# SAR-Research-Lab/lvt

Hardware: AMD Instinct MI355X
Metric: stereo frames/sec (KITTI-shaped 1241x376), per-frame SE3 vs CPU ref (higher is better)
Workload: dtype u8/f64

## Files before the change

include/lvt_amd_ext.h:

```cpp
#ifndef LVT_AMD_EXT_H__
#define LVT_AMD_EXT_H__

#include "lvt_c.h"
#include <stdint.h>

#ifdef __cplusplus
extern "C" {
#endif

typedef struct lvt_amd_params {
    float fx, fy, cx, cy;
    float baseline;
    int img_width, img_height;
    float k1, k2, p1, p2, k3;
    float near_plane_distance, far_plane_distance;
    float triangulation_ratio_test_threshold;
    float tracking_ratio_test_threshold;
    float descriptor_matching_threshold;
    int min_num_matches_for_tracking;
    int tracking_radius;
    int detection_cell_size;
    int max_keypoints_per_cell;
    int agast_threshold;
    int untracked_threshold;
// ... 34 lines not shown
LVT_API void lvt_amd_batch_track_device_async(lvt_handle h, const void *const *d_left, const void *const *d_right,
                                              int n_rows, int n_cols, int pitch_bytes);
LVT_API void lvt_amd_batch_wait(lvt_handle h, double *R, double *t, int *status);
LVT_API void lvt_amd_batch_get_counts(lvt_handle h, int seq, int out[32]);
LVT_API lvt_handle lvt_amd_batch_create_mixed(const lvt_amd_params *p , int sensor_type, int n_sequences);
LVT_API int lvt_amd_batch_track_device_async_mixed(lvt_handle h, const void *const *d_left, const void *const *d_right,
                                                   const int *n_rows, const int *n_cols, const int *pitch_bytes);
LVT_API int lvt_amd_batch_get_params(lvt_handle h, int seq, lvt_amd_params *out);
LVT_API int lvt_amd_batch_mixed_tables(const lvt_amd_params *p, int sensor_type, int n_sequences, unsigned *cells, int cells_cap,
                                       unsigned *score, int score_cap, int counts[2]);

LVT_API void lvt_amd_set_stream(lvt_handle h, void *hip_stream);
LVT_API const char *lvt_amd_last_error(lvt_handle h);

LVT_API void lvt_amd_get_host_stats(lvt_handle h, long long out[8]);

LVT_API void lvt_amd_profile_enable(lvt_handle h, int enable);
LVT_API int lvt_amd_profile_read(lvt_handle h, int slot, char *name, int name_cap, double *total_ms, long *calls);

enum {
    LVT_AMD_C_N_LEFT = 0, LVT_AMD_C_N_RIGHT, LVT_AMD_C_MAP_SIZE, LVT_AMD_C_STAGED_SIZE, LVT_AMD_C_N_MATCHES,
    LVT_AMD_C_SECOND_PASS, LVT_AMD_C_N_ROW_MATCHES, LVT_AMD_C_N_TRIANGULATED, LVT_AMD_C_TRIANGULATED,
    LVT_AMD_C_RETRY_LEFT, LVT_AMD_C_RETRY_RIGHT, LVT_AMD_C_PNP_ITERS, LVT_AMD_C_PNP_INLIERS,
    LVT_AMD_C_MAP_SIZE_AT_MATCH, LVT_AMD_C_N_STAGED_ERASED, LVT_AMD_C_N_STAGED_PROMOTED, LVT_AMD_C_N_CULLED,
    LVT_AMD_C_FRAME, LVT_AMD_C_OVERFLOW ,
    LVT_AMD_C_PNP_BORDERLINE ,
    LVT_AMD_C_ROW_FALLBACK ,
    LVT_AMD_C_PNP_TRIALS , LVT_AMD_C_PNP_REJECTIONS ,
    LVT_AMD_C_PNP_TERMINATES ,
    LVT_AMD_C__COUNT = 32
};
LVT_API void lvt_amd_get_counts(lvt_handle h, int out[LVT_AMD_C__COUNT]);
LVT_API int lvt_amd_get_features(lvt_handle h, int eye, float *xy, float *resp, uint8_t *desc, int cap);
LVT_API int lvt_amd_get_matches(lvt_handle h, int *feat_idx, double *xyz, int cap);
LVT_API int lvt_amd_get_row_matches(lvt_handle h, int *pairs, int cap);
LVT_API int lvt_amd_get_map(lvt_handle h, double *xyz, int *counter, int *age, uint8_t *desc, int cap);
LVT_API int lvt_amd_get_staged(lvt_handle h, double *xyz, int *counter, uint8_t *desc, int cap);
enum { LVT_AMD_LISTS_MAP = 0, LVT_AMD_LISTS_STAGED = 1, LVT_AMD_LISTS_ROW = 2 };
typedef struct {
    int kc;
    int stood_down_map;
    int stood_down_row;
    int pass2;
    int n_early;
    int binned;
    int n;
    int reserved;
} lvt_amd_list_info;
LVT_API int lvt_amd_get_candidate_lists(lvt_handle h, int which, unsigned *keys, int *counts, float *proj, signed char *vis, int cap, lvt_amd_list_info *info);
LVT_API void lvt_amd_get_pose(lvt_handle h, double q_wxyz[4], double p[3]);
LVT_API int lvt_amd_get_last_pose(lvt_handle h, double q_wxyz[4], double p[3]);
LVT_API void lvt_amd_get_predicted_pose(lvt_handle h, double q_wxyz[4], double p[3]);
LVT_API void lvt_amd_get_debug(lvt_handle h, long long out[32]);
LVT_API void lvt_amd_get_timeline(lvt_handle h, long long out[16]);
LVT_API int lvt_amd_get_ordering(lvt_handle h);
LVT_API int lvt_amd_get_plane(lvt_handle h, int eye, int what, void *dst, int cap_bytes, int *pitch_out);

LVT_API int lvt_amd_pnp(const lvt_amd_params *p, const double q_in[4], const double p_in[3], const double *pts,
                        const float *obs, int n, double q_out[4], double p_out[3], int *n_solve_calls);
LVT_API int lvt_amd_pnp_detail(const lvt_amd_params *p, const double q_in[4], const double p_in[3], const double *pts,
                               const float *obs, int n, double q_out[4], double p_out[3], int *n_solve_calls,
                               double *err_out, int *level_out, int *borderline);
LVT_API int lvt_amd_pnp_trace(const lvt_amd_params *p, const double q_in[4], const double p_in[3], const double *pts,
                              const float *obs, int n, double q_out[4], double p_out[3], int *n_solve_calls,
                              double *err_out, int *level_out, int *borderline, double *trace, int trace_cap, int stats[3]);
LVT_API int lvt_amd_motion_predict(double state[14], const double q[4], const double p[3], double q_out[4], double p_out[3]);
// ... 177 lines not shown
```

lvt_amd/__init__.py:

```python
from __future__ import annotations

import ctypes as C
import os

import numpy as np

from .params import LvtParameters, ParamsPOD, kitti_params, euroc_params, tum_params

_HERE = os.path.dirname(os.path.abspath(__file__))
LIB_PATH = os.environ.get("LVT_AMD_LIB") or os.path.join(_HERE, "lib", "liblvt_c.so")

ABI_SYMBOLS = [
    "lvt_create", "lvt_destroy", "lvt_track", "lvt_track_with_external_corners", "lvt_get_status",
    "lvt_amd_default_params", "lvt_amd_params_from_file", "lvt_amd_create", "lvt_amd_reset",
    "lvt_amd_track_rgbd", "lvt_amd_track_device", "lvt_amd_track_device_async", "lvt_amd_wait",
    "lvt_amd_set_stream", "lvt_amd_last_error", "lvt_amd_get_counts", "lvt_amd_get_features",
    "lvt_amd_get_matches", "lvt_amd_get_row_matches", "lvt_amd_get_map", "lvt_amd_get_staged", "lvt_amd_get_candidate_lists",
    "lvt_amd_get_pose", "lvt_amd_get_last_pose", "lvt_amd_get_predicted_pose", "lvt_amd_get_plane", "lvt_amd_pnp", "lvt_amd_pnp_detail",
    "lvt_amd_hamming_match_batched", "lvt_amd_hamming_match_batched_n", "lvt_amd_rectifier_create", "lvt_amd_rectifier_destroy",
    "lvt_amd_rectify_device", "lvt_amd_rectify", "lvt_amd_rectifier_get_maps",
    "lvt_amd_odometry_create", "lvt_amd_odometry_destroy", "lvt_amd_odometry_reset", "lvt_amd_odometry_push_pose", "lvt_amd_odometry_update", "lvt_amd_profile_enable", "lvt_amd_profile_read", "lvt_amd_get_debug", "lvt_amd_get_timeline", "lvt_amd_get_ordering",
    "lvt_amd_batch_create", "lvt_amd_batch_size", "lvt_amd_batch_track_device_async", "lvt_amd_batch_wait",
    "lvt_amd_batch_get_counts", "lvt_amd_create_on_device", "lvt_amd_get_device", "lvt_amd_wait_status", "lvt_amd_get_host_stats",
    "lvt_amd_track_async", "lvt_amd_track_rgbd_async", "lvt_amd_pnp_trace", "lvt_amd_create_pooled", "lvt_amd_wait_pose",
    "lvt_amd_batch_create_mixed", "lvt_amd_batch_track_device_async_mixed", "lvt_amd_batch_get_params", "lvt_amd_batch_mixed_tables",
    "lvt_amd_track_rgbd_device", "lvt_amd_track_rgbd_device_async", "lvt_amd_track_rgbd16", "lvt_amd_track_rgbd16_async",
    "lvt_amd_batch_track_rgbd_device_async",
    "lvt_amd_set_rectifiers", "lvt_amd_batch_set_rectifiers",
    "lvt_amd_set_pixel_format", "lvt_amd_batch_set_pixel_format", "lvt_amd_get_pixel_format",
    "lvt_amd_motion_predict",
    "lvt_amd_snapshot_take", "lvt_amd_snapshot_apply", "lvt_amd_batch_snapshot_take", "lvt_amd_batch_snapshot_apply", "lvt_amd_snapshot_get_info",
    "lvt_amd_snapshot_get_params", "lvt_amd_snapshot_export", "lvt_amd_snapshot_import", "lvt_amd_snapshot_describe", "lvt_amd_snapshot_destroy",
    "lvt_amd_batch_reset",
    "lvt_amd_enable_pose_info", "lvt_amd_get_pose_info", "lvt_amd_pose_info_eval", "lvt_amd_pose_info_to_ros",
    "lvt_amd_odometry_push_pose_cov", "lvt_amd_odometry_update_cov",
    "lvt_amd_set_depth_camera", "lvt_amd_batch_set_depth_camera", "lvt_amd_get_depth_camera", "lvt_amd_register_depth_device",
    "lvt_amd_set_equalisation", "lvt_amd_batch_set_equalisation", "lvt_amd_get_equalisation", "lvt_amd_equalise_device", "lvt_amd_equalisation_plan",
    "lvt_amd_set_mask", "lvt_amd_batch_set_mask", "lvt_amd_set_mask_device", "lvt_amd_batch_set_mask_device", "lvt_amd_get_mask_stats", "lvt_amd_mask_features",
    "lvt_amd_set_label_mask", "lvt_amd_batch_set_label_mask", "lvt_amd_get_label_mask", "lvt_amd_frame_labels", "lvt_amd_frame_labels_device", "lvt_amd_build_label_mask",
    "lvt_amd_depth_guard_default", "lvt_amd_set_depth_guard", "lvt_amd_batch_set_depth_guard", "lvt_amd_get_depth_guard", "lvt_amd_get_depth_guard_stats", "lvt_amd_depth_guard_features",
    "lvt_amd_relocalise", "lvt_amd_batch_relocalise", "lvt_amd_odometry_set_relocalisation", "lvt_amd_reloc_default_config", "lvt_amd_reloc_slice_length", "lvt_amd_reloc_match_device", "lvt_amd_reloc_solve", "lvt_amd_reloc_correspond",
]

N_COUNTS = 32
COUNT_NAMES = ["n_left", "n_right", "map_size", "staged_size", "n_matches", "second_pass", "n_row_matches",
               "n_triangulated", "triangulated", "retry_left", "retry_right", "pnp_iters", "pnp_inliers",
               "map_size_at_match", "n_staged_erased", "n_staged_promoted", "n_culled", "frame", "overflow", "pnp_borderline", "row_fallback", "pnp_trials", "pnp_rejections", "pnp_terminates"]

LISTS_WHICH = {"map": 0, "staged": 1, "row": 2}
LIST_INFO_NAMES = ["kc", "stood_down_map", "stood_down_row", "pass2", "n_early", "binned", "n"]

eState_NOT_INITIALIZED, eState_TRACKING, eState_LOST = 1, 2, 3
eSensor_STEREO, eSensor_RGBD = 1, 2
PIX_GRAY8, PIX_BGR8, PIX_RGB8, PIX_BGRA8, PIX_RGBA8 = 0, 1, 2, 3, 4
PIX_BPP = {PIX_GRAY8: 1, PIX_BGR8: 3, PIX_RGB8: 3, PIX_BGRA8: 4, PIX_RGBA8: 4}
DEPTH_F32, DEPTH_U16 = 0, 1

_lib = None


def load_library():
    global _lib
    if _lib is not None:
        return _lib
    if not os.path.exists(LIB_PATH):
        raise RuntimeError(f"{LIB_PATH} is missing: build it with `make -C lvt_amd/csrc` "
                           "(there is no CPU fallback for the tracking path)")
    try:
        import torch
    except Exception:
        pass
    L = C.CDLL(LIB_PATH)
    vp = C.c_void_p
    L.lvt_create.restype = vp
    L.lvt_create.argtypes = [C.c_char_p, C.c_int]
    L.lvt_amd_create.restype = vp
    L.lvt_amd_create.argtypes = [vp, C.c_int]
    L.lvt_amd_create_on_device.restype = vp
    L.lvt_amd_create_on_device.argtypes = [vp, C.c_int, C.c_int]
    L.lvt_amd_get_device.argtypes = [vp]
    L.lvt_amd_create_pooled.restype = vp
    L.lvt_amd_create_pooled.argtypes = [vp, C.c_int, C.c_int]
    L.lvt_destroy.argtypes = [vp]
    L.lvt_amd_reset.argtypes = [vp]
    L.lvt_track.argtypes = [vp, vp, vp, C.c_int, C.c_int, vp, vp]
    L.lvt_track_with_external_corners.argtypes = [vp, vp, vp, C.c_int, C.c_int, vp, C.c_int, vp, C.c_int, vp, vp]
    L.lvt_get_status.argtypes = [vp]
    L.lvt_amd_params_from_file.argtypes = [C.c_char_p, vp]
    L.lvt_amd_default_params.argtypes = [vp]
    L.lvt_amd_track_rgbd.argtypes = [vp, vp, vp, C.c_int, C.c_int, vp, vp]
    L.lvt_amd_track_device.argtypes = [vp, vp, vp, C.c_int, C.c_int, C.c_int, vp, vp]
    L.lvt_amd_track_device_async.argtypes = [vp, vp, vp, C.c_int, C.c_int, C.c_int]
    L.lvt_amd_wait.argtypes = [vp, vp, vp]
    L.lvt_amd_track_async.argtypes = [vp, vp, vp, C.c_int, C.c_int]
    L.lvt_amd_track_async.restype = C.c_int
    L.lvt_amd_track_rgbd_async.argtypes = [vp, vp, vp, C.c_int, C.c_int]
    L.lvt_amd_track_rgbd_async.restype = C.c_int
    L.lvt_amd_wait_status.argtypes = [vp, vp, vp]
    L.lvt_amd_wait_status.restype = C.c_int
    L.lvt_amd_set_stream.argtypes = [vp, vp]
    L.lvt_amd_last_error.restype = C.c_char_p
    L.lvt_amd_last_error.argtypes = [vp]
    L.lvt_amd_get_counts.argtypes = [vp, vp]
    L.lvt_amd_get_features.argtypes = [vp, C.c_int, vp, vp, vp, C.c_int]
    L.lvt_amd_get_matches.argtypes = [vp, vp, vp, C.c_int]
    L.lvt_amd_get_row_matches.argtypes = [vp, vp, C.c_int]
    L.lvt_amd_get_map.argtypes = [vp, vp, vp, vp, vp, C.c_int]
    L.lvt_amd_get_staged.argtypes = [vp, vp, vp, vp, C.c_int]
    L.lvt_amd_get_candidate_lists.argtypes = [vp, C.c_int, vp, vp, vp, vp, C.c_int, vp]
    L.lvt_amd_get_candidate_lists.restype = C.c_int
    L.lvt_amd_get_pose.argtypes = [vp, vp, vp]
    L.lvt_amd_get_last_pose.argtypes = [vp, vp, vp]
    L.lvt_amd_get_predicted_pose.argtypes = [vp, vp, vp]
    L.lvt_amd_get_plane.argtypes = [vp, C.c_int, C.c_int, vp, C.c_int, vp]
    L.lvt_amd_pnp.argtypes = [vp, vp, vp, vp, vp, C.c_int, vp, vp, vp]
    L.lvt_amd_pnp_detail.argtypes = [vp, vp, vp, vp, vp, C.c_int, vp, vp, vp, vp, vp, vp]
    L.lvt_amd_pnp_trace.argtypes = [vp, vp, vp, vp, vp, C.c_int, vp, vp, vp, vp, vp, vp, vp, C.c_int, vp]
    L.lvt_amd_motion_predict.argtypes = [vp, vp, vp, vp, vp]
    L.lvt_amd_motion_predict.restype = C.c_int
    L.lvt_amd_hamming_match_batched.restype = C.c_float
    L.lvt_amd_hamming_match_batched.argtypes = [vp, vp, vp, vp, vp, C.c_int, C.c_int, C.c_int, C.c_float, C.c_int, C.c_int, C.c_int, vp, vp]
    L.lvt_amd_get_timeline.argtypes = [vp, vp]
    L.lvt_amd_get_ordering.argtypes = [vp]
    L.lvt_amd_get_ordering.restype = C.c_int
    L.lvt_amd_rectifier_create.restype = vp
    L.lvt_amd_rectifier_create.argtypes = [vp, vp, vp, vp, C.c_int, C.c_int]
    L.lvt_amd_rectifier_destroy.argtypes = [vp]
    L.lvt_amd_rectify_device.argtypes = [vp, vp, C.c_int, vp, C.c_int, vp]
    L.lvt_amd_rectify.argtypes = [vp, vp, vp]
    L.lvt_amd_rectifier_get_maps.argtypes = [vp, vp, vp]
    L.lvt_amd_odometry_create.restype = vp
    L.lvt_amd_odometry_create.argtypes = [vp, vp, C.c_int]
    L.lvt_amd_odometry_destroy.argtypes = [vp]
    L.lvt_amd_odometry_reset.argtypes = [vp]
    L.lvt_amd_odometry_push_pose.restype = C.c_int
    L.lvt_amd_odometry_push_pose.argtypes = [vp, vp, vp, C.c_int, C.c_double, vp, vp]
    L.lvt_amd_odometry_update.restype = C.c_int
# ... 813 lines not shown
        return _depth_guard_of(self._h, 0)

    def depth_guard_stats(self):
        return _depth_guard_stats_of(self._h, 0)

    def _depth(self, d):
        want = getattr(self, "_depth_shape", None)
        if want is not None and tuple(d.shape) != want:
            raise ValueError(f"a depth image of shape {tuple(d.shape)} on a system whose depth camera delivers {want}")
        return d

    def depth_camera(self):
        return _depth_camera_of(self._h, 0)

    def enable_pose_info(self, on: bool = True) -> int:
        return load_library().lvt_amd_enable_pose_info(self._h, 1 if on else 0)

    def pose_info(self) -> PoseInfo:
        return _pose_info_of(self._h, 0)

    def set_stream(self, hip_stream: int):
        load_library().lvt_amd_set_stream(self._h, C.c_void_p(hip_stream))

    def counts(self):
        a = np.zeros(N_COUNTS, dtype=np.int32)
        load_library().lvt_amd_get_counts(self._h, _p(a))
        return {n: int(a[i]) for i, n in enumerate(COUNT_NAMES)}

    def features(self, eye=0, cap=16384):
        xy = np.zeros((cap, 2), np.float32); resp = np.zeros(cap, np.float32); desc = np.zeros((cap, 32), np.uint8)
        n = load_library().lvt_amd_get_features(self._h, eye, _p(xy), _p(resp), _p(desc), cap)
        return xy[:n].copy(), resp[:n].copy(), desc[:n].copy()

    def matches(self, cap=65536):
        fi = np.zeros(cap, np.int32); xyz = np.zeros((cap, 3), np.float64)
        n = load_library().lvt_amd_get_matches(self._h, _p(fi), _p(xyz), cap)
        return fi[:n].copy(), xyz[:n].copy()

    def row_matches(self, cap=16384):
        pr = np.zeros((cap, 2), np.int32)
        n = load_library().lvt_amd_get_row_matches(self._h, _p(pr), cap)
        return pr[:n].copy()

    def map(self, cap=65536):
        xyz = np.zeros((cap, 3)); cnt = np.zeros(cap, np.int32); age = np.zeros(cap, np.int32); desc = np.zeros((cap, 32), np.uint8)
        n = load_library().lvt_amd_get_map(self._h, _p(xyz), _p(cnt), _p(age), _p(desc), cap)
        return xyz[:n].copy(), cnt[:n].copy(), age[:n].copy(), desc[:n].copy()

    def staged(self, cap=65536):
        xyz = np.zeros((cap, 3)); cnt = np.zeros(cap, np.int32); desc = np.zeros((cap, 32), np.uint8)
        n = load_library().lvt_amd_get_staged(self._h, _p(xyz), _p(cnt), _p(desc), cap)
        return xyz[:n].copy(), cnt[:n].copy(), desc[:n].copy()

    def candidate_lists(self, which, cap=None):
        w = LISTS_WHICH[which] if isinstance(which, str) else int(which)
        L = load_library()
        info = np.zeros(8, np.int32)
        if cap is None:
            L.lvt_amd_get_candidate_lists(self._h, w, None, None, None, None, 0, _p(info))
            cap = int(info[6])
        kc = 128
        keys = np.zeros((max(cap, 1), kc), np.uint32); counts = np.zeros(max(cap, 1), np.int32)
        proj = np.zeros((max(cap, 1), 2), np.float32); vis = np.zeros(max(cap, 1), np.int8)
        n = L.lvt_amd_get_candidate_lists(self._h, w, _p(keys), _p(counts), _p(proj), _p(vis), cap, _p(info))
        if n < 0:
            raise ValueError("lvt_amd_get_candidate_lists refused the call (bad handle, a batch, `which` out of range, or cap too small)")
# ... 407 lines not shown
```

lvt_amd/csrc/k_features.hip:

```cpp
#include "lvt_dev.h"
#include "lvt_handover.h"
#include "lvt_math.h"
#include <type_traits>

namespace lvt {

__constant__ signed char c_brief[256][4] = {
#include "../../include/lvt_brief256_pattern.inc"
};
constexpr signed char BRIEF_TABLE[256][4] = {
#include "../../include/lvt_brief256_pattern.inc"
};
constexpr int brief_max_offset() {
    int m = 0;
    for (int i = 0; i < 256; i++)
        for (int k = 0; k < 4; k++) m = (BRIEF_TABLE[i][k] > m) ? BRIEF_TABLE[i][k] : (-BRIEF_TABLE[i][k] > m) ? -BRIEF_TABLE[i][k] : m;
    return m;
}

constexpr int TS_W = 64, TS_H = 16, HALO = 4;
constexpr int TILE_W = TS_W + 2 * HALO;
constexpr int TILE_H = TS_H + 2 * HALO;

typedef short s16x2 __attribute__((ext_vector_type(2)));
// ... 1621 lines not shown
    const int n_out = anms_select<uint16_t>(S, c.g, L, n, out, nullptr);
    cell_finish(FB, eye, cell, 0, n_out);
}

__device__ __forceinline__ bool brief_border_keep(float x, float y, int rows, int cols) {
    const int B = 28;
    if (rows <= 2 * B || cols <= 2 * B) return false;
    const int ix = __float2int_rn(x), iy = __float2int_rn(y);
    return ix >= B && ix < cols - B && iy >= B && iy < rows - B;
}

template <bool BV>
__global__ __launch_bounds__(1024) void k_gather(SeqArg<BV> sa, int par) {
    const Seq &S = sa.get();
    const int eye = blockIdx.y;
    const FrameBuf &FB = S.fb[par];
    FeatCtl &ctl = *FB.fc;
    extern __shared__ __attribute__((aligned(16))) uint8_t smem[];
    const CellLds L = carve_cell_lds(smem);
    int *cell_off = L.row_first;
    int *scan = L.scan;
    const int tid = threadIdx.x;
    const Feat &F = FB.feat[eye];
    if (ctl.poison) return;
    if (!ctl.ext_corners && !(eye == 1 && S.prm.sensor == 2) && ctl.n_detected[eye] < CORNERS_LOW_TH) {
        for (int cell = 0; cell < S.prm.n_cells; cell++) {
            cells_work(S, FB, eye, cell, 1, L);
            __syncthreads();
        }
        __builtin_amdgcn_fence(__ATOMIC_RELEASE, "workgroup");
        __syncthreads();
        __builtin_amdgcn_fence(__ATOMIC_ACQUIRE, "workgroup");
    }
    if (eye == 1 && S.prm.sensor == 2) {
        if (tid == 0) *F.n = 0;
        return;
    }
    const FrameIn &in = ctl.in;
    const bool rgbd = (S.prm.sensor == 2);
    const float *ext_xy = nullptr, *depth_img = nullptr;
    int depth_pitch = 0, depth_format = DEPTH_F32;
    float depth_scale = 0.f;
    if (ctl.ext_corners) ext_xy = wave_uniform(in.ext_xy[eye]);
    if (rgbd) {
        depth_img = wave_uniform(in.depth_img);
        depth_pitch = wave_uniform(in.depth_pitch), depth_format = wave_uniform(in.depth_format);
        depth_scale = wave_uniform(in.depth_scale);
    }
    const int nc = ctl.ext_corners ? 1 : S.prm.n_cells;
    if (tid == 0) {
        int acc = 0;
        for (int c = 0; c < nc; c++) {
            cell_off[c] = acc;
            acc += ctl.ext_corners ? ctl.n_ext[eye] : FB.cell_n[eye][c];
        }
        cell_off[nc] = acc;
    }
    __syncthreads();
    const int total_in = cell_off[nc];
    const int W = S.prm.W, H = S.prm.H;
    int n_out = 0;
    for (int base = 0; base < total_in; base += 1024) {
        const int g = base + tid;
        bool keep = false;
        float x = 0, y = 0, r = 0, ox = 0, oy = 0, dep = 0;
        if (g < total_in) {
            if (ctl.ext_corners) {
                x = ext_xy[2 * g];
                y = ext_xy[2 * g + 1];
            } else {
                int c = 0;
                while (g >= cell_off[c + 1]) c++;
                const float *kp = FB.cell_kp[eye] + ((size_t)c * CELL_OUT_CAP + (g - cell_off[c])) * 3;
                x = kp[0];
                y = kp[1];
                r = kp[2];
            }
            ox = x;
            oy = y;
            keep = brief_border_keep(x, y, H, W);
            if (keep && rgbd) {
                const size_t di = (size_t)((int)y) * depth_pitch + (int)x;
                dep = depth_sample(depth_img, depth_format, depth_scale, di);
                keep = (dep >= S.prm.near_plane && dep <= S.prm.far_plane);
                if (keep && S.prm.undistort) {
                    undistort_point(S.prm, x, y, x, y);
                    const int hy = (int)floorf(y / (float)HASH_CELL), hx = (int)floorf(x / (float)HASH_CELL);
                    if (hy < 0 || hy >= S.prm.hash_ccy || hx < 0 || hx >= S.prm.hash_ccx) keep = false;
                }
            }
        }
        int total;
        const int off = n_out + block_excl_scan(keep ? 1 : 0, scan, &total);
        if (keep && off < NF_MAX) {
            F.x[off] = x;
            F.y[off] = y;
            F.resp[off] = r;
            F.bx[off] = ox;
            F.by[off] = oy;
            F.depth[off] = dep;
            F.flag[off] = 0;
            F.hcy[off] = (int16_t)floorf(y / (float)HASH_CELL);
            F.hcx[off] = (int16_t)floorf(x / (float)HASH_CELL);
        }
        n_out += total;
    }
    if (tid == 0) {
        if (n_out > NF_MAX) {
            atomicOr(&ctl.overflow, OVF_FEATURES);
            n_out = NF_MAX;
        }
        *F.n = n_out;
    }
}

__device__ __forceinline__ int box_at(const Seq &S, const FrameBuf &FB, int eye, int iy, int ix) {
    const int W = S.prm.W, H = S.prm.H;
    if (ix >= 0 && ix < W && iy >= 0 && iy < H) return FB.boxsum[eye][(size_t)iy * S.plane_pitch + ix];
    const FrameIn &in = FB.fc->in;
    int s = 0;
    for (int y = max(iy - 4, 0); y <= min(iy + 4, H - 1); y++)
        for (int x = max(ix - 4, 0); x <= min(ix + 4, W - 1); x++) s += in.img[eye][(size_t)y * in.img_pitch + x];
    return s;
}

__device__ __forceinline__ int brief_plane_of_block(int &plane, int &bx) {
    const int planes = gridDim.y * gridDim.z;
    int lid = blockIdx.x + gridDim.x * (blockIdx.y + gridDim.y * blockIdx.z);
    plane = lid / gridDim.x, bx = lid % gridDim.x;
    if ((planes & 7) == 0) {
        const int j = lid >> 3;
        plane = (lid & 7) + 8 * (j / gridDim.x);
        bx = j % gridDim.x;
    }
    return planes;
}
__device__ __forceinline__ int brief_key_points_of_wave(int planes, int bx, int wpb, int n, int &i, int &i_end) {
    int stride = gridDim.x * wpb;
    i = bx * wpb + wave_id();
// ... 228 lines not shown
```

lvt_amd/csrc/k_track.hip:

```cpp
#include "lvt_dev.h"
#include "lvt_handover.h"
#include "wave_reduce.h"
#include "lvt_math.h"

namespace lvt {

enum : int { MODE_MAP = 0, MODE_STAGED = 1, MODE_ROW = 2 };

__device__ __forceinline__ void frame_prologue(const Seq &S, Ctl &c, int par, const Pose &predicted, const double mm_next[14], bool active,
                                               bool first, bool skipped) {
    const bool absent = skipped && S.fb[par].fc->absent != 0;
    if (!absent) {
        for (int i = 0; i < N_COUNTS; i++) c.counts[i] = 0;
        c.counts[C_FRAME] = c.frame_number;
        c.frame_number++;
    }
    c.active = active ? 1 : 0;
    c.first_frame = first ? 1 : 0;
    c.do_pass2 = 0;
    c.n_pass1 = c.n_pass2 = 0;
    c.n_matches = 0;
    c.lost_now = 0;
    c.need_tri = 0;
    c.dont_stage = 0;
// ... 121 lines not shown
    int M;
    const uint64_t *qdesc;
    uint32_t *cand;
    int *ncand;
    if (MODE == MODE_MAP) {
        M = *S.map_n;
        qdesc = S.map[*S.map_cur].desc;
        cand = S.cand;
        ncand = S.ncand;
    } else if (MODE == MODE_STAGED) {
        M = *S.staged_n;
        qdesc = S.staged[*S.staged_cur].desc;
        cand = S.scand;
        ncand = S.sncand;
    } else {
        M = *S.fb[par].feat[0].n;
        qdesc = S.fb[par].feat[0].desc;
        cand = S.rcand + (size_t)par * NF_MAX * KC;
        ncand = S.rncand + par * NF_MAX;
    }
    if (q_end >= 0) M = min(M, q_end);
    wave0 += q_begin;
    if (wave0 - wv >= M) return;
    uint64_t qd0[4] = {0, 0, 0, 0};
    double X0[3] = {0, 0, 0};
    if (wave0 < M) {
#pragma unroll
        for (int k = 0; k < 4; k++) qd0[k] = qdesc[(size_t)wave0 * 4 + k];
        if (MODE == MODE_MAP && PROJECT) {
            const MapSoA &P0 = S.map[*S.map_cur];
            X0[0] = P0.pos[3 * wave0], X0[1] = P0.pos[3 * wave0 + 1], X0[2] = P0.pos[3 * wave0 + 2];
        }
    }
    {
        const int t0 = PROJECT ? (int)threadIdx.x - 64 : (int)threadIdx.x, tn = PROJECT ? nthreads - 64 : nthreads;
        if (t0 >= 0)
            for (int j0 = t0; j0 < N; j0 += 4 * tn) {
                float vx[4], vy[4];
                int16_t cy[4], cx[4];
#pragma unroll
                for (int k = 0; k < 4; k++) {
                    const int j = min(j0 + k * tn, N - 1);
                    vx[k] = T.x[j], vy[k] = T.y[j];
                    if (MODE != MODE_ROW) cy[k] = T.hcy[j], cx[k] = T.hcx[j];
                }
#pragma unroll
                for (int k = 0; k < 4; k++) {
                    const int j = j0 + k * tn;
                    if (j < N) {
                        s_tx[j] = vx[k];
                        s_ty[j] = vy[k];
                        if (MODE != MODE_ROW) s_tc[j] = ((uint32_t)(uint16_t)cy[k] << 16) | (uint32_t)(uint16_t)cx[k];
                    }
                }
            }
    }
    __syncthreads();
    const int radius = S.prm.tracking_radius * ((MODE == MODE_MAP && pass2) ? 2 : 1);
    uint32_t *buf = C.lbuf + wv * KC;
    for (int i = wave0; i < M; i += wave_stride) {
        Query q;
        if (MODE == MODE_MAP && PROJECT) {
            const MapSoA &P = S.map[*S.map_cur];
            double X[3] = {X0[0], X0[1], X0[2]};
            if (i != wave0) X[0] = P.pos[3 * i], X[1] = P.pos[3 * i + 1], X[2] = P.pos[3 * i + 2];
            double u, v;
            const bool visible = is_point_visible(X, C.w2c, S.prm, u, v);
            if (lane == 0) {
                if (visible) {
                    S.proj[2 * i] = (float)u;
                    S.proj[2 * i + 1] = (float)v;
                    S.vis[i] = 1;
                    S.match[i] = -1;
                } else {
                    S.vis[i] = 0;
                    P.counter[i] += 1;
                    S.match[i] = -2;
                    ncand[i] = 0;
                }
            }
            if (!visible) continue;
            make_query_track(S.prm, (float)u, (float)v, radius, q);
        } else if (MODE == MODE_MAP) {
            if (!S.vis[i]) {
                if (lane == 0) ncand[i] = 0;
                continue;
            }
            make_query_track(S.prm, S.proj[2 * i], S.proj[2 * i + 1], radius, q);
        } else if (MODE == MODE_STAGED) {
            if (!S.svis[i]) {
                if (lane == 0) ncand[i] = 0;
                continue;
            }
            make_query_track(S.prm, S.sproj[2 * i], S.sproj[2 * i + 1], radius, q);
        } else {
            make_query_row(S.prm, S.fb[par].feat[0].x[i], S.fb[par].feat[0].y[i], q);
        }
#pragma unroll
        for (int k = 0; k < 4; k++) q.d[k] = (i == wave0) ? qd0[k] : qdesc[(size_t)i * 4 + k];
        int cnt = 0;
        uint32_t c_n = 0;
        float x_n = 0.f, y_n = 0.f;
        {
            const int j0 = min(lane, NF_MAX - 1);
            y_n = s_ty[j0];
            if (MODE != MODE_ROW) c_n = s_tc[j0], x_n = s_tx[j0];
        }
        for (int base = 0; base < N; base += 64) {
            const int j = base + lane;
            const uint32_t c = c_n;
            const float fx = x_n, fy = y_n;
            {
                const int jn = min(j + 64, NF_MAX - 1);
                y_n = s_ty[jn];
                if (MODE != MODE_ROW) c_n = s_tc[jn], x_n = s_tx[jn];
            }
            bool ok = false;
            if (j < N) {
                if (MODE == MODE_ROW) {
                    ok = fy >= (float)q.sy && fy <= (float)q.ey;
                } else {
                    const int cy = (int)(int16_t)(c >> 16), cx = (int)(int16_t)(c & 0xFFFFu);
                    if (cy >= q.sy && cy < q.ey && cx >= q.sx && cx < q.ex) {
                        const float dx = fx - q.x, dy = fy - q.y;
                        ok = (dx * dx + dy * dy) < q.r2;
                    }
                }
            }
            const uint64_t m = __ballot(ok);
            if (ok) {
                const int pos = cnt + __popcll(m & lt_mask);
                if (pos < KC) buf[pos] = (uint32_t)j;
            }
            cnt += __popcll(m);
        }
        __builtin_amdgcn_fence(__ATOMIC_ACQ_REL, "workgroup");
        if (cnt <= KC) {
            for (int e = lane; e < cnt; e += 64) {
                const uint32_t j = buf[e];
                uint64_t t[4];
#pragma unroll
                for (int k = 0; k < 4; k++) t[k] = T.desc[(size_t)j * 4 + k];
                buf[e] = ((uint32_t)hamming256(q.d, t) << 16) | j;
            }
            __builtin_amdgcn_fence(__ATOMIC_ACQ_REL, "workgroup");
            for (int e = lane; e < cnt; e += 64) {
                const uint32_t k = buf[e];
                int rank = 0;
                for (int o = 0; o < cnt; o++) rank += (buf[o] < k) ? 1 : 0;
                cand[(size_t)i * KC + rank] = k;
            }
// ... 1694 lines not shown
```

lvt_amd/csrc/lvt_dev.h:

```cpp
#pragma once
#include <hip/hip_runtime.h>
#include <stdint.h>

namespace lvt {

constexpr int NF_MAX = 4096;
constexpr int CELLS_MAX = 64;
constexpr int CELL_OUT_CAP = 2048;
constexpr int RAW_CAP = 10240;
constexpr int CELL_SIDE_LDS = 1024;
constexpr int CELL_SIDE_MAX = 4096;
constexpr int BIG_CELL_SIDE = 256;
constexpr int MAP_MAX = 32768;
constexpr int STAGED_MAX = 16384;
constexpr int KC = 128;
constexpr int N_COUNTS = 32;

enum : int { OVF_RAW = 1, OVF_CELL_OUT = 2, OVF_FEATURES = 4, OVF_MAP = 8, OVF_STAGED = 16, OVF_CELL_DIM = 32 };

enum : int {
    C_N_LEFT = 0, C_N_RIGHT, C_MAP_SIZE, C_STAGED_SIZE, C_N_MATCHES, C_SECOND_PASS, C_N_ROW_MATCHES,
    C_N_TRIANGULATED, C_TRIANGULATED, C_RETRY_LEFT, C_RETRY_RIGHT, C_PNP_ITERS, C_PNP_INLIERS,
    C_MAP_SIZE_AT_MATCH, C_N_STAGED_ERASED, C_N_STAGED_PROMOTED, C_N_CULLED, C_FRAME, C_OVERFLOW, C_PNP_BORDERLINE,
    C_ROW_FALLBACK,
// ... 68 lines not shown

constexpr int NPAR = 3;

enum { DEPTH_F32 = 0, DEPTH_U16 = 1 };

struct FrameIn {
    const uint8_t *img[2];
    const float *depth_img;
    int img_pitch, depth_pitch;
    int depth_format;
    float depth_scale;
    const float *ext_xy[2];
};

struct FeatCtl {
    int ext_corners;
    int n_ext[2];
    int n_detected[2];
    int retry[2];
    int overflow;
    seq_t row_seq;
    unsigned done_blocks;
    int absent;
    int poison;
    seq_t skip_seq;
    seq_t feat_seq;
    FrameIn in;
    int lost_n[2];
    seq_t lost_seq;
    int mask_kept[2], mask_dropped[2];
    int guard_kept, guard_dropped;
};

struct Feat {
    float *x, *y, *resp;
    float *bx, *by;
    float *depth;
    uint64_t *desc;
    uint8_t *flag;
    int16_t *hcx, *hcy;
    int *n;
};

struct MapSoA {
    double *pos;
    uint64_t *desc;
    int *counter, *age, *match_idx;
};

struct FrameBuf {
    uint8_t *score[2];
    uint16_t *boxsum[2];
    uint32_t *seg_keys[2];
    uint16_t *seg_cnt[2];
    float *cell_kp[2];
    int *cell_n[2];
    const float *ext_xy_own[2];
    Feat feat[2];
    FeatCtl *fc;
};

enum { LFB_MAP = 0, LFB_ROW = 1, LFB_EARLY_N = 2 ,
       LFB_STAGED_N = 3 , LFB_WORDS = 4 };

struct Seq {
    Params prm;
    Ctl *ctl;
    FrameBuf fb[NPAR];
    int plane_pitch;
    uint32_t *cell_scratch[2];
    size_t cell_scratch_off[CELLS_MAX];
    uint32_t *strip_kp[2];
    int *strip_n[2];
    int *cell_big[2];
// ... 41 lines not shown
}

__device__ __forceinline__ int wave_incl_scan(int v) {
    v += __builtin_amdgcn_update_dpp(0, v, 0x111, 0xf, 0xf, false);
    v += __builtin_amdgcn_update_dpp(0, v, 0x112, 0xf, 0xf, false);
    v += __builtin_amdgcn_update_dpp(0, v, 0x114, 0xf, 0xf, false);
    v += __builtin_amdgcn_update_dpp(0, v, 0x118, 0xf, 0xf, false);
    v += __builtin_amdgcn_update_dpp(0, v, 0x142, 0xa, 0xf, false);
    v += __builtin_amdgcn_update_dpp(0, v, 0x143, 0xc, 0xf, false);
    return v;
}
__device__ __forceinline__ int row16_incl_scan(int v) {
    v += __builtin_amdgcn_update_dpp(0, v, 0x111, 0xf, 0xf, false);
    v += __builtin_amdgcn_update_dpp(0, v, 0x112, 0xf, 0xf, false);
    v += __builtin_amdgcn_update_dpp(0, v, 0x114, 0xf, 0xf, false);
    v += __builtin_amdgcn_update_dpp(0, v, 0x118, 0xf, 0xf, false);
    return v;
}

__device__ __forceinline__ int block_excl_scan(int v, int *scratch, int *total) {
    const int incl = wave_incl_scan(v);
    const int w = __builtin_amdgcn_readfirstlane(wave_id()), l = lane_id();
    const int nw = (blockDim.x + 63) >> 6;
    __syncthreads();
    if (l == 63) scratch[w] = incl;
    __syncthreads();
    const int part = (l < nw) ? scratch[l] : 0;
    const int pin = row16_incl_scan(part);
    const int base = __builtin_amdgcn_readlane(pin, w) - __builtin_amdgcn_readlane(part, w);
    *total = __builtin_amdgcn_readlane(pin, 15);
    return base + incl - v;
}

template <typename Keep>
__device__ __forceinline__ int compact_features(const Feat &F, int *scan, int *n_before, Keep keep_of) {
    const int tid = threadIdx.x;
    const int n_in = min(max(*F.n, 0), NF_MAX);
    int n_out = 0;
    for (int base = 0; base < n_in; base += 1024) {
        const int g = base + tid;
        bool keep = false;
        float x = 0, y = 0, r = 0, bx = 0, by = 0, dep = 0;
        int16_t hcx = 0, hcy = 0;
        if (g < n_in) {
            x = F.x[g], y = F.y[g], r = F.resp[g];
            bx = F.bx[g], by = F.by[g];
            dep = F.depth[g];
            hcx = F.hcx[g], hcy = F.hcy[g];
            keep = keep_of(bx, by);
        }
        int total;
        const int off = n_out + block_excl_scan(keep ? 1 : 0, scan, &total);
        if (keep && off != g) {
            F.x[off] = x, F.y[off] = y, F.resp[off] = r;
            F.bx[off] = bx, F.by[off] = by;
            F.depth[off] = dep;
            F.hcx[off] = hcx, F.hcy[off] = hcy;
        }
        n_out += total;
    }
    if (tid == 0) *F.n = n_out;
    *n_before = n_in;
    return n_out;
}

__device__ __forceinline__ float depth_sample(const float *img, int fmt, float scale, size_t i) {
    return (fmt == DEPTH_U16) ? __fmul_rn((float)reinterpret_cast<const uint16_t *>(img)[i], scale) : img[i];
}

template <bool BYVAL>
struct SeqArg;
typedef const __attribute__((address_space(4))) Seq *SeqConstPtr;
__device__ __forceinline__ const Seq &seq_const(const Seq *p, unsigned i) { return *(const Seq *)((SeqConstPtr)p + i); }
template <>
struct SeqArg<false> {
    const Seq *p;
    __device__ __forceinline__ const Seq &get() const { return seq_const(p, blockIdx.z); }
    __device__ __forceinline__ const Seq &at(unsigned i) const { return seq_const(p, i); }
};
template <>
struct SeqArg<true> {
    Seq v;
    __device__ __forceinline__ const Seq &get() const { return v; }
    __device__ __forceinline__ const Seq &at(unsigned) const { return v; }
};
constexpr size_t KERNARG_MAX = 4096, BYVAL_REST_MAX = 256;
static_assert(sizeof(SeqArg<true>) + BYVAL_REST_MAX <= KERNARG_MAX, "a by-value Seq and the arguments behind it must fit the kernel-argument segment");


}
```

lvt_amd/csrc/lvt_host.hip:

```cpp
#define LVT_EXPORT_FUNCTIONS
#include "../../include/lvt_amd_ext.h"

#include "k_features.hip"
#include "k_track.hip"
#include "k_hamming.hip"
#include "k_lists.hip"
#include "k_rectify.hip"
#include "k_depthreg.hip"
#include "k_equalise.hip"
#include "k_depthguard.hip"
#include "k_mask.hip"
#include "k_labelmask.hip"
#include "k_state.hip"
#include "k_poseinfo.hip"
#include "k_reloc.hip"
#include "lvt_odometry.h"

#include <atomic>
#include <cmath>
#include <chrono>
#include <cstdio>
#include <cstdlib>
#include <cstring>
#include <string>
// ... 405 lines not shown
    auto get = [&](const char *k) -> double {
        for (auto &e : kv)
            if (e.first == k) return e.second;
        return 0.0;
    };
    auto geti = [&](const char *k) -> int { return (int)std::nearbyint(get(k)); };
    p->fx = (float)get("fx"), p->fy = (float)get("fy"), p->cx = (float)get("cx"), p->cy = (float)get("cy");
    p->k1 = (float)get("k1"), p->k2 = (float)get("k2"), p->p1 = (float)get("p1"), p->p2 = (float)get("p2"), p->k3 = (float)get("k3");
    p->baseline = (float)get("baseline");
    p->img_width = geti("img_width"), p->img_height = geti("img_height");
    p->near_plane_distance = (float)get("near_plane_distance");
    p->far_plane_distance = (float)get("far_plane_distance");
    p->triangulation_ratio_test_threshold = (float)get("triangulation_ratio_test_threshold");
    p->tracking_ratio_test_threshold = (float)get("tracking_ratio_test_threshold");
    p->min_num_matches_for_tracking = geti("min_num_matches_for_tracking");
    p->tracking_radius = geti("tracking_radius");
    p->agast_threshold = geti("agast_threshold");
    p->untracked_threshold = geti("untracked_threshold");
    p->staged_threshold = geti("staged_threshold");
    p->descriptor_matching_threshold = (float)get("descriptor_matching_threshold");
    p->detection_cell_size = geti("detection_cell_size");
    p->max_keypoints_per_cell = geti("max_keypoints_per_cell");
    p->triangulation_policy = geti("triangulation_policy");
    return true;
}

static void alloc_feat(Context *c, Feat &F) {
    F.x = c->dalloc<float>(NF_MAX), F.y = c->dalloc<float>(NF_MAX), F.resp = c->dalloc<float>(NF_MAX);
    F.bx = c->dalloc<float>(NF_MAX), F.by = c->dalloc<float>(NF_MAX), F.depth = c->dalloc<float>(NF_MAX);
    F.desc = c->dalloc<uint64_t>((size_t)NF_MAX * 4);
    F.flag = c->dalloc<uint8_t>(NF_MAX);
    F.hcx = c->dalloc<int16_t>(NF_MAX), F.hcy = c->dalloc<int16_t>(NF_MAX);
    F.n = c->dalloc<int>(1);
}
static void alloc_points(Context *c, MapSoA &P, int cap) {
    P.pos = c->dalloc<double>((size_t)cap * 3);
    P.desc = c->dalloc<uint64_t>((size_t)cap * 4);
    P.counter = c->dalloc<int>(cap), P.age = c->dalloc<int>(cap), P.match_idx = c->dalloc<int>(cap);
}

static void drain(Context *c);

static void pose_info_clear(Context *c, int s) {
    if (!c->h_pinfo) return;
    for (int r = 0; r < RING; r++) std::memset(&c->h_pinfo[(size_t)r * c->B + s], 0, sizeof(lvt_amd_pose_info));
}
static Ctl fresh_ctl(const Context *c) {
    Ctl z;
    std::memset(&z, 0, sizeof(z));
    z.state = 1;
    z.last_matches[0] = z.last_matches[1] = z.last_matches[2] = 0x7FFFFFFF;
    z.last_pose.q[0] = 1.0;
    z.mm_last_q[0] = 1.0;
    z.mm_ang_vel[0] = 1.0;
    z.optimized.q[0] = z.predicted.q[0] = 1.0;
    z.out_R[0] = z.out_R[4] = z.out_R[8] = 1.0;
    z.out_status = 1;
    z.pnp_seq = (seq_t)c->enq;
    z.early_state = early_word((seq_t)c->enq, EARLY_NOTHING);
    z.track_done_seq = (seq_t)c->enq;
    z.late_gate_seq = (seq_t)c->enq;
    z.gate_timeouts = c->gate_timeouts_seen, z.gate_fatal = c->gate_fatal_seen;
    return z;
}
static void reset_state(Context *c, int only = -1) {
    drain(c);
// ... 1663 lines not shown
}

LVT_API void lvt_amd_get_counts(lvt_handle h, int out[LVT_AMD_C__COUNT]) {
    h = resolve_handle(h);
    try {
        View v;
        if (!view_of(h, v)) return;
        for (int i = 0; i < LVT_AMD_C__COUNT; i++) out[i] = v.rec->counts[i];
    } catch (...) {
    }
}

LVT_API int lvt_amd_get_features(lvt_handle h, int eye, float *xy, float *resp, uint8_t *desc, int cap) {
    h = resolve_handle(h);
    try {
        View v;
        if (!view_of(h, v)) return -1;
        Context *c = v.c;
        const Feat &F = c->h_seqs[v.s].fb[v.par].feat[eye ? 1 : 0];
        const int n = read_scalar(c, F.n), m = std::min(n, cap);
        std::vector<float> x(m), y(m);
        d2h(c, x.data(), F.x, m);
        d2h(c, y.data(), F.y, m);
        if (xy)
            for (int i = 0; i < m; i++) xy[2 * i] = x[i], xy[2 * i + 1] = y[i];
        d2h(c, resp, F.resp, m);
        d2h(c, desc, reinterpret_cast<const uint8_t *>(F.desc), (size_t)m * 32);
        return n;
    } catch (...) {
    }
    return -1;
}

LVT_API int lvt_amd_get_matches(lvt_handle h, int *feat_idx, double *xyz, int cap) {
    h = resolve_handle(h);
    try {
        View v;
        if (!view_of(h, v)) return -1;
        Context *c = v.c;
        const int n = v.rec->n_matches, m = std::min(n, cap);
        d2h(c, feat_idx, c->h_seqs[v.s].pnp_feat, m);
        d2h(c, xyz, c->h_seqs[v.s].pnp_X, (size_t)m * 3);
        return n;
    } catch (...) {
    }
    return -1;
}

LVT_API int lvt_amd_get_row_matches(lvt_handle h, int *pairs, int cap) {
    h = resolve_handle(h);
    try {
        View v;
        if (!view_of(h, v)) return -1;
        Context *c = v.c;
        const int n = v.rec->counts[C_N_ROW_MATCHES], m = std::min(n, cap);
        std::vector<int> l(m), r(m);
        d2h(c, l.data(), c->h_seqs[v.s].pair_l, m);
        d2h(c, r.data(), c->h_seqs[v.s].pair_r, m);
        for (int i = 0; i < m; i++) pairs[2 * i] = l[i], pairs[2 * i + 1] = r[i];
        return n;
    } catch (...) {
    }
    return -1;
}

static int get_points(Context *c, const MapSoA *bufs, const int *d_cur, const int *d_n, double *xyz, int *counter, int *age, uint8_t *desc,
// ... 835 lines not shown
```

Measured before the change: 9146.

## Record per-cell feature range bounds and skip unreachable feature spans in tracking

Feature detection and compaction now keep, for each detection cell, a table of feature index range, hash-cell bounds and y bounds. The table is built with DPP segmented scans and LDS atomics. The tracking kernel loads this table one range per lane, ballots which ranges can overlap the query window, and walks only those merged index spans instead of scanning all N features in 64-wide steps. This is meant to cut candidate-search work per map point or row query, at the cost of extra scan and atomic work during feature output and compaction plus per-query readlane control logic. A validity check falls back to a full scan when the table is inconsistent.

```diff
diff --git a/include/lvt_amd_ext.h b/include/lvt_amd_ext.h
--- a/include/lvt_amd_ext.h
+++ b/include/lvt_amd_ext.h
@@ -90,6 +90,13 @@
 };
 LVT_API void lvt_amd_get_counts(lvt_handle h, int out[LVT_AMD_C__COUNT]);
 LVT_API int lvt_amd_get_features(lvt_handle h, int eye, float *xy, float *resp, uint8_t *desc, int cap);
+enum { LVT_AMD_RANGES_MAX = 64 };
+typedef struct {
+    int first[LVT_AMD_RANGES_MAX], count[LVT_AMD_RANGES_MAX];
+    short hcx_min[LVT_AMD_RANGES_MAX], hcx_max[LVT_AMD_RANGES_MAX], hcy_min[LVT_AMD_RANGES_MAX], hcy_max[LVT_AMD_RANGES_MAX];
+    float y_min[LVT_AMD_RANGES_MAX], y_max[LVT_AMD_RANGES_MAX];
+} lvt_amd_feature_ranges;
+LVT_API int lvt_amd_get_feature_ranges(lvt_handle h, int eye, lvt_amd_feature_ranges *out);
 LVT_API int lvt_amd_get_matches(lvt_handle h, int *feat_idx, double *xyz, int cap);
 LVT_API int lvt_amd_get_row_matches(lvt_handle h, int *pairs, int cap);
 LVT_API int lvt_amd_get_map(lvt_handle h, double *xyz, int *counter, int *age, uint8_t *desc, int cap);
diff --git a/lvt_amd/__init__.py b/lvt_amd/__init__.py
--- a/lvt_amd/__init__.py
+++ b/lvt_amd/__init__.py
@@ -14,7 +14,7 @@
     "lvt_create", "lvt_destroy", "lvt_track", "lvt_track_with_external_corners", "lvt_get_status",
     "lvt_amd_default_params", "lvt_amd_params_from_file", "lvt_amd_create", "lvt_amd_reset",
     "lvt_amd_track_rgbd", "lvt_amd_track_device", "lvt_amd_track_device_async", "lvt_amd_wait",
-    "lvt_amd_set_stream", "lvt_amd_last_error", "lvt_amd_get_counts", "lvt_amd_get_features",
+    "lvt_amd_set_stream", "lvt_amd_last_error", "lvt_amd_get_counts", "lvt_amd_get_features", "lvt_amd_get_feature_ranges",
     "lvt_amd_get_matches", "lvt_amd_get_row_matches", "lvt_amd_get_map", "lvt_amd_get_staged", "lvt_amd_get_candidate_lists",
     "lvt_amd_get_pose", "lvt_amd_get_last_pose", "lvt_amd_get_predicted_pose", "lvt_amd_get_plane", "lvt_amd_pnp", "lvt_amd_pnp_detail",
     "lvt_amd_hamming_match_batched", "lvt_amd_hamming_match_batched_n", "lvt_amd_rectifier_create", "lvt_amd_rectifier_destroy",
@@ -49,6 +49,11 @@
 
 LISTS_WHICH = {"map": 0, "staged": 1, "row": 2}
 LIST_INFO_NAMES = ["kc", "stood_down_map", "stood_down_row", "pass2", "n_early", "binned", "n"]
+
+RANGES_MAX = 64
+RANGES_DTYPE = np.dtype([("first", np.int32, RANGES_MAX), ("count", np.int32, RANGES_MAX),
+                         ("hcx_min", np.int16, RANGES_MAX), ("hcx_max", np.int16, RANGES_MAX), ("hcy_min", np.int16, RANGES_MAX), ("hcy_max", np.int16, RANGES_MAX),
+                         ("y_min", np.float32, RANGES_MAX), ("y_max", np.float32, RANGES_MAX)])
 
 eState_NOT_INITIALIZED, eState_TRACKING, eState_LOST = 1, 2, 3
 eSensor_STEREO, eSensor_RGBD = 1, 2
@@ -103,6 +108,8 @@
     L.lvt_amd_last_error.argtypes = [vp]
     L.lvt_amd_get_counts.argtypes = [vp, vp]
     L.lvt_amd_get_features.argtypes = [vp, C.c_int, vp, vp, vp, C.c_int]
+    L.lvt_amd_get_feature_ranges.argtypes = [vp, C.c_int, vp]
+    L.lvt_amd_get_feature_ranges.restype = C.c_int
     L.lvt_amd_get_matches.argtypes = [vp, vp, vp, C.c_int]
     L.lvt_amd_get_row_matches.argtypes = [vp, vp, C.c_int]
     L.lvt_amd_get_map.argtypes = [vp, vp, vp, vp, vp, C.c_int]
@@ -982,6 +989,16 @@
         n = load_library().lvt_amd_get_features(self._h, eye, _p(xy), _p(resp), _p(desc), cap)
         return xy[:n].copy(), resp[:n].copy(), desc[:n].copy()
 
+    def feature_ranges(self, eye=0):
+        raw = np.zeros(1, RANGES_DTYPE)
+        n = load_library().lvt_amd_get_feature_ranges(self._h, eye, _p(raw))
+        if n < 0:
+            raise ValueError("lvt_amd_get_feature_ranges refused the call")
+        out = np.zeros(RANGES_MAX, [(k, RANGES_DTYPE[k].base) for k in RANGES_DTYPE.names])
+        for k in RANGES_DTYPE.names:
+            out[k] = raw[k][0]
+        return out, n
+
     def matches(self, cap=65536):
         fi = np.zeros(cap, np.int32); xyz = np.zeros((cap, 3), np.float64)
         n = load_library().lvt_amd_get_matches(self._h, _p(fi), _p(xyz), cap)
diff --git a/lvt_amd/csrc/k_features.hip b/lvt_amd/csrc/k_features.hip
--- a/lvt_amd/csrc/k_features.hip
+++ b/lvt_amd/csrc/k_features.hip
@@ -1677,8 +1677,13 @@
         __syncthreads();
         __builtin_amdgcn_fence(__ATOMIC_ACQUIRE, "workgroup");
     }
+    RangeAcc &acc = *reinterpret_cast<RangeAcc *>(L.row_end);
+    static_assert(sizeof(RangeAcc) <= 1024 * sizeof(int), "the range accumulators live in CellLds::row_end");
+    range_acc_clear(acc, tid);
     if (eye == 1 && S.prm.sensor == 2) {
         if (tid == 0) *F.n = 0;
+        __syncthreads();
+        if (tid < CELLS_MAX && F.rng) range_acc_store(acc, F.rng, tid);
         return;
     }
     const FrameIn &in = ctl.in;
@@ -1709,12 +1714,13 @@
         const int g = base + tid;
         bool keep = false;
         float x = 0, y = 0, r = 0, ox = 0, oy = 0, dep = 0;
+        int c = nc - 1;
         if (g < total_in) {
+            c = 0;
             if (ctl.ext_corners) {
                 x = ext_xy[2 * g];
                 y = ext_xy[2 * g + 1];
             } else {
-                int c = 0;
                 while (g >= cell_off[c + 1]) c++;
                 const float *kp = FB.cell_kp[eye] + ((size_t)c * CELL_OUT_CAP + (g - cell_off[c])) * 3;
                 x = kp[0];
@@ -1735,6 +1741,7 @@
                 }
             }
         }
+        range_acc_add(acc, keep, c, (int16_t)floorf(x / (float)HASH_CELL), (int16_t)floorf(y / (float)HASH_CELL), y);
         int total;
         const int off = n_out + block_excl_scan(keep ? 1 : 0, scan, &total);
         if (keep && off < NF_MAX) {
@@ -1750,6 +1757,7 @@
         }
         n_out += total;
     }
+    if (tid < CELLS_MAX && F.rng) range_acc_store(acc, F.rng, tid, n_out > NF_MAX);
     if (tid == 0) {
         if (n_out > NF_MAX) {
             atomicOr(&ctl.overflow, OVF_FEATURES);
diff --git a/lvt_amd/csrc/k_track.hip b/lvt_amd/csrc/k_track.hip
--- a/lvt_amd/csrc/k_track.hip
+++ b/lvt_amd/csrc/k_track.hip
@@ -177,6 +177,19 @@
             X0[0] = P0.pos[3 * wave0], X0[1] = P0.pos[3 * wave0 + 1], X0[2] = P0.pos[3 * wave0 + 2];
         }
     }
+    int rg_first = 0, rg_count = -1, rg_a = 0, rg_b = 0;
+    {
+        const FeatRanges *R = T.rng;
+        if (R) {
+            rg_first = R->first[lane], rg_count = R->count[lane];
+            if (MODE == MODE_ROW) {
+                rg_a = __float_as_int(R->y_min[lane]), rg_b = __float_as_int(R->y_max[lane]);
+            } else {
+                rg_a = (int)((uint32_t)(uint16_t)R->hcx_min[lane] | (uint32_t)(uint16_t)R->hcx_max[lane] << 16);
+                rg_b = (int)((uint32_t)(uint16_t)R->hcy_min[lane] | (uint32_t)(uint16_t)R->hcy_max[lane] << 16);
+            }
+        }
+    }
     {
         const int t0 = PROJECT ? (int)threadIdx.x - 64 : (int)threadIdx.x, tn = PROJECT ? nthreads - 64 : nthreads;
         if (t0 >= 0)
@@ -201,6 +214,8 @@
             }
     }
     __syncthreads();
+    const bool rg_use = range_table_valid(rg_first, rg_count, N);
+    const uint32_t rg_fc = rg_use ? (uint32_t)rg_first | (uint32_t)rg_count << 16 : (lane == 0 ? (uint32_t)N << 16 : 0u);
     const int radius = S.prm.tracking_radius * ((MODE == MODE_MAP && pass2) ? 2 : 1);
     uint32_t *buf = C.lbuf + wv * KC;
     for (int i = wave0; i < M; i += wave_stride) {
@@ -246,22 +261,52 @@
         int cnt = 0;
         uint32_t c_n = 0;
         float x_n = 0.f, y_n = 0.f;
+        uint64_t sel = 0;
         {
-            const int j0 = min(lane, NF_MAX - 1);
+            bool reach = (rg_fc >> 16) != 0;
+            if (rg_use) {
+                if (MODE == MODE_ROW) {
+                    reach = reach && !(__int_as_float(rg_b) < (float)q.sy || __int_as_float(rg_a) > (float)q.ey);
+                } else {
+                    const int x0 = (int)(int16_t)rg_a, x1 = rg_a >> 16, y0 = (int)(int16_t)rg_b, y1 = rg_b >> 16;
+                    reach = reach && !(x1 < q.sx || x0 >= q.ex || y1 < q.sy || y0 >= q.ey);
+                }
+            }
+            sel = __ballot(reach);
+        }
+        int nb = 0, ne = 0;
+        auto next_trip = [&]() -> bool {
+            nb += 64;
+            if (nb < ne) return true;
+            if (!sel) return false;
+            uint32_t fc = (uint32_t)__builtin_amdgcn_readlane((int)rg_fc, (int)__builtin_ctzll(sel));
+            sel &= sel - 1;
+            nb = (int)(fc & 0xFFFFu), ne = nb + (int)(fc >> 16);
+            while (sel) {
+                fc = (uint32_t)__builtin_amdgcn_readlane((int)rg_fc, (int)__builtin_ctzll(sel));
+                if ((int)(fc & 0xFFFFu) != ne) break;
+                ne += (int)(fc >> 16), sel &= sel - 1;
+            }
+            return true;
+        };
+        bool more = next_trip();
+        if (more) {
+            const int j0 = min(nb + lane, NF_MAX - 1);
             y_n = s_ty[j0];
             if (MODE != MODE_ROW) c_n = s_tc[j0], x_n = s_tx[j0];
         }
-        for (int base = 0; base < N; base += 64) {
-            const int j = base + lane;
+        while (more) {
+            const int j = nb + lane, end = ne;
             const uint32_t c = c_n;
             const float fx = x_n, fy = y_n;
-            {
-                const int jn = min(j + 64, NF_MAX - 1);
+            more = next_trip();
+            if (more) {
+                const int jn = min(nb + lane, NF_MAX - 1);
                 y_n = s_ty[jn];
                 if (MODE != MODE_ROW) c_n = s_tc[jn], x_n = s_tx[jn];
             }
             bool ok = false;
-            if (j < N) {
+            if (j < end) {
                 if (MODE == MODE_ROW) {
                     ok = fy >= (float)q.sy && fy <= (float)q.ey;
                 } else {
diff --git a/lvt_amd/csrc/lvt_dev.h b/lvt_amd/csrc/lvt_dev.h
--- a/lvt_amd/csrc/lvt_dev.h
+++ b/lvt_amd/csrc/lvt_dev.h
@@ -124,6 +124,13 @@
     int guard_kept, guard_dropped;
 };
 
+struct FeatRanges {
+    int first[CELLS_MAX], count[CELLS_MAX];
+    int16_t hcx_min[CELLS_MAX], hcx_max[CELLS_MAX], hcy_min[CELLS_MAX], hcy_max[CELLS_MAX];
+    float y_min[CELLS_MAX], y_max[CELLS_MAX];
+};
+static_assert(CELLS_MAX == 64, "a wavefront holds the range table one range per lane");
+
 struct Feat {
     float *x, *y, *resp;
     float *bx, *by;
@@ -132,6 +139,7 @@
     uint8_t *flag;
     int16_t *hcx, *hcy;
     int *n;
+    FeatRanges *rng;
 };
 
 struct MapSoA {
@@ -239,23 +247,107 @@
     return base + incl - v;
 }
 
+__device__ __forceinline__ int float_order_key(float f) {
+    const int u = __float_as_int(f);
+    return u ^ ((u >> 31) & 0x7FFFFFFF);
+}
+__device__ __forceinline__ float float_of_order_key(int k) { return __int_as_float(k ^ ((k >> 31) & 0x7FFFFFFF)); }
+
+__device__ __forceinline__ bool range_table_valid(int first, int count, int n) {
+    const int incl = wave_incl_scan(count);
+    const bool bad = count < 0 || (count > 0 && incl - count != first);
+    return __ballot(bad) == 0 && __builtin_amdgcn_readlane(incl, 63) == n;
+}
+
+struct RangeAcc {
+    int count[CELLS_MAX], hcx_min[CELLS_MAX], hcx_max[CELLS_MAX], hcy_min[CELLS_MAX], hcy_max[CELLS_MAX], y_min[CELLS_MAX], y_max[CELLS_MAX];
+};
+__device__ __forceinline__ void range_acc_clear(RangeAcc &A, int tid) {
+    if (tid < CELLS_MAX) {
+        A.count[tid] = 0;
+        A.hcx_min[tid] = A.hcy_min[tid] = 32767, A.hcx_max[tid] = A.hcy_max[tid] = -32768;
+        A.y_min[tid] = float_order_key(INFINITY), A.y_max[tid] = float_order_key(-INFINITY);
+    }
+}
+typedef short rg_short2 __attribute__((ext_vector_type(2)));
+__device__ __forceinline__ int pk_min_i16(int a, int b) {
+    return __builtin_bit_cast(int, __builtin_elementwise_min(__builtin_bit_cast(rg_short2, a), __builtin_bit_cast(rg_short2, b)));
+}
+__device__ __forceinline__ int pk_max_i16(int a, int b) {
+    return __builtin_bit_cast(int, __builtin_elementwise_max(__builtin_bit_cast(rg_short2, a), __builtin_bit_cast(rg_short2, b)));
+}
+template <int CTRL>
+__device__ __forceinline__ void range_scan_step(int r, int &hmin, int &hmax, int &fmin, int &fmax) {
+    const bool same = __builtin_amdgcn_update_dpp(-1, r, CTRL, 0xf, 0xf, false) == r;
+    const int a = __builtin_amdgcn_update_dpp(hmin, hmin, CTRL, 0xf, 0xf, false), b = __builtin_amdgcn_update_dpp(hmax, hmax, CTRL, 0xf, 0xf, false);
+    const int c = __builtin_amdgcn_update_dpp(fmin, fmin, CTRL, 0xf, 0xf, false), d = __builtin_amdgcn_update_dpp(fmax, fmax, CTRL, 0xf, 0xf, false);
+    if (same) hmin = pk_min_i16(hmin, a), hmax = pk_max_i16(hmax, b), fmin = min(fmin, c), fmax = max(fmax, d);
+}
+__device__ __forceinline__ void range_acc_add(RangeAcc &A, bool on, int r, int hcx, int hcy, float y) {
+    const int hc = (int)((uint32_t)(uint16_t)hcx | (uint32_t)(uint16_t)hcy << 16);
+    int hmin = on ? hc : 0x7FFF7FFF, hmax = on ? hc : (int)0x80008000;
+    int fmin = (on && y == y) ? float_order_key(y) : 0x7FFFFFFF, fmax = (on && y == y) ? float_order_key(y) : (int)0x80000000;
+    const int p = (int)__popcll(__ballot(on) & lanes_below(lane_id()));
+    const bool head = __builtin_amdgcn_update_dpp(-1, r, 0x111, 0xf, 0xf, false) != r;
+    const bool tail = __builtin_amdgcn_update_dpp(-1, r, 0x101, 0xf, 0xf, false) != r;
+    range_scan_step<0x111>(r, hmin, hmax, fmin, fmax);
+    range_scan_step<0x112>(r, hmin, hmax, fmin, fmax);
+    range_scan_step<0x114>(r, hmin, hmax, fmin, fmax);
+    range_scan_step<0x118>(r, hmin, hmax, fmin, fmax);
+    if (r >= 0 && r < CELLS_MAX) {
+        if (head && p) atomicSub(&A.count[r], p);
+        if (tail) {
+            atomicAdd(&A.count[r], p + (on ? 1 : 0));
+            atomicMin(&A.hcx_min[r], (int)(int16_t)hmin), atomicMax(&A.hcx_max[r], (int)(int16_t)hmax);
+            atomicMin(&A.hcy_min[r], hmin >> 16), atomicMax(&A.hcy_max[r], hmax >> 16);
+            atomicMin(&A.y_min[r], fmin), atomicMax(&A.y_max[r], fmax);
+        }
+    }
+}
+__device__ __forceinline__ void range_acc_store(const RangeAcc &A, FeatRanges *R, int tid, bool give_up = false) {
+    const int cnt = give_up ? -1 : A.count[tid];
+    R->first[tid] = wave_incl_scan(cnt) - cnt;
+    R->count[tid] = cnt;
+    R->hcx_min[tid] = (int16_t)A.hcx_min[tid], R->hcx_max[tid] = (int16_t)A.hcx_max[tid];
+    R->hcy_min[tid] = (int16_t)A.hcy_min[tid], R->hcy_max[tid] = (int16_t)A.hcy_max[tid];
+    R->y_min[tid] = float_of_order_key(A.y_min[tid]), R->y_max[tid] = float_of_order_key(A.y_max[tid]);
+}
+
 template <typename Keep>
 __device__ __forceinline__ int compact_features(const Feat &F, int *scan, int *n_before, Keep keep_of) {
     const int tid = threadIdx.x;
     const int n_in = min(max(*F.n, 0), NF_MAX);
+    FeatRanges *R = F.rng;
+    __shared__ RangeAcc acc;
+    __shared__ int r_end[CELLS_MAX];
+    if (R) {
+        if (tid < CELLS_MAX) {
+            const int first = R->first[tid], count = R->count[tid];
+            const int incl = wave_incl_scan(max(count, 0));
+            r_end[tid] = range_table_valid(first, count, n_in) ? incl : n_in;
+        }
+        range_acc_clear(acc, tid);
+        __syncthreads();
+    }
     int n_out = 0;
     for (int base = 0; base < n_in; base += 1024) {
         const int g = base + tid;
         bool keep = false;
         float x = 0, y = 0, r = 0, bx = 0, by = 0, dep = 0;
         int16_t hcx = 0, hcy = 0;
+        int rg = CELLS_MAX - 1;
         if (g < n_in) {
+            rg = 0;
             x = F.x[g], y = F.y[g], r = F.resp[g];
             bx = F.bx[g], by = F.by[g];
             dep = F.depth[g];
             hcx = F.hcx[g], hcy = F.hcy[g];
             keep = keep_of(bx, by);
+            if (R)
+                for (int s = CELLS_MAX / 2; s; s >>= 1)
+                    if (g >= r_end[rg + s - 1]) rg += s;
         }
+        if (R) range_acc_add(acc, keep, rg, hcx, hcy, y);
         int total;
         const int off = n_out + block_excl_scan(keep ? 1 : 0, scan, &total);
         if (keep && off != g) {
@@ -266,6 +358,7 @@
         }
         n_out += total;
     }
+    if (R && tid < CELLS_MAX) range_acc_store(acc, R, tid);
     if (tid == 0) *F.n = n_out;
     *n_before = n_in;
     return n_out;
diff --git a/lvt_amd/csrc/lvt_host.hip b/lvt_amd/csrc/lvt_host.hip
--- a/lvt_amd/csrc/lvt_host.hip
+++ b/lvt_amd/csrc/lvt_host.hip
@@ -461,6 +461,7 @@
     F.flag = c->dalloc<uint8_t>(NF_MAX);
     F.hcx = c->dalloc<int16_t>(NF_MAX), F.hcy = c->dalloc<int16_t>(NF_MAX);
     F.n = c->dalloc<int>(1);
+    F.rng = c->dalloc<FeatRanges>(1);
 }
 static void alloc_points(Context *c, MapSoA &P, int cap) {
     P.pos = c->dalloc<double>((size_t)cap * 3);
@@ -2190,6 +2191,22 @@
     return -1;
 }
 
+static_assert(sizeof(lvt_amd_feature_ranges) == sizeof(FeatRanges) && LVT_AMD_RANGES_MAX == CELLS_MAX, "lvt_amd_feature_ranges is FeatRanges");
+LVT_API int lvt_amd_get_feature_ranges(lvt_handle h, int eye, lvt_amd_feature_ranges *out) {
+    h = resolve_handle(h);
+    try {
+        View v;
+        if (!out || !view_of(h, v)) return -1;
+        Context *c = v.c;
+        const Feat &F = c->h_seqs[v.s].fb[v.par].feat[eye ? 1 : 0];
+        const int n = read_scalar(c, F.n);
+        d2h(c, reinterpret_cast<FeatRanges *>(out), F.rng, 1);
+        return n;
+    } catch (...) {
+    }
+    return -1;
+}
+
 LVT_API int lvt_amd_get_matches(lvt_handle h, int *feat_idx, double *xyz, int cap) {
     h = resolve_handle(h);
     try {
```

New measurement: 8868. -3.0%, worse.
